# Grice-Lab/HmmUFOtu

Measured on AMD Instinct MI355X. Metric: reads placed/sec (whole node), gg_97_otus GTR+dGamma 250bp; HBM GB/s %peak, higher is better.
Workload: dtype f64; 1 GPU; gg_97_otus-scale synthetic DB (198643 nodes x 7682 CS columns, K=1400), GTR+dGamma(4), SE 250 bp amplicon reads, batch 8192 reads/step/GPU, 6 batches in flight, seeds in the reference's std::sort order (k_seed_refsort); seed_order=reference, message_window_cols=7682, parallelism=read-sharded x1

## Files before the change

### hmmufotu_amd/csrc/hu_common.h

```cpp
#pragma once
#include <hip/hip_runtime.h>
#include <stdint.h>
#include <string>
#include <functional>
#include <istream>
#include <ostream>
#include <vector>
#include <exception>
#include <mutex>
#include <thread>
#include "../../include/hmmufotu_amd.h"

#define HU_MAX_DGK 16
#define HU_READ_TILE 16
#define HU_MAX_INS 24
#define HU_NODE_PAD 256
#define HU_MIN_LOGLIK_EXP (-510.0)
#define HU_BRANCH_EPS 1e-5
#define HU_MAX_ITER 100

struct HuModelDev {
	int32_t type, dgK;
	double pi[4];
	double logpi[4];
	double U[16], U1[16], lam[4];
	double rate[HU_MAX_DGK];
};

struct HuDbDev {
	int32_t nNodes, nNodesPad, csLen, W, WQ, root;
	int64_t winStart, winLen;
	const uint4* planes;
	const int32_t* posCol;
	const unsigned long long* colPlanes;
	int32_t QM, pad0;
	const uint2* nodeCover;
	const int32_t* parent;
	const double* blen;
	const double* height;
	const double* up;
	const double* down;
	const int32_t* upK;
	const int32_t* downK;
	int32_t K, L;
	const double* EM;
	const double* EI;
	const double* T;
	const double* entryC;
	const double* exitC;
	const int32_t* p2cs;
	const double* Tt;
	const double* EMt;
	const double* EIt;
	const double* placeConst;
	int32_t rLo, rHi;
	const uint32_t* wideList;
};
__device__ inline bool hu_skip_width(const HuDbDev& db, int cols) { return db.rHi != 0 && (cols <= db.rLo || cols > db.rHi); }

struct HuRegion {
	int32_t j0, j1, i0, i1;
	int32_t withB;
	int32_t band;
	int32_t from, start, nIns, nDel;
	int64_t off;
	int64_t doff;
	int32_t ci0, cj0;
	int64_t coff;
};
// ... 75 lines not shown
```

### hmmufotu_amd/csrc/hu_engine.hip

```cpp
#include <algorithm>
#include <cmath>
#include <cstdio>
#include <cstring>
#include <limits>
#include <map>
#include <atomic>
#include <thread>
#include <memory>
#include <mutex>
#include <chrono>
#include <fstream>
#include <sstream>
#include <new>
#include <stdexcept>
#include <fcntl.h>
#include <unistd.h>
#include "hu_common.h"
#include "hu_kern_sep.h"
#include "hu_kern_align.h"
#include "hu_kern_tree.h"
#include "hu_kern_blk.h"
#include "hu_kern_refsort.h"
#include "hu_kern_rank.h"
#include "hu_kern_anneal.h"
// ... 90 lines not shown
			for(size_t i = 0; i < v.size(); ++i) if(v[i] == (void*) p) { v.erase(v.begin() + i); free(p); return; }
		}
		(void) hipHostFree(p);
	}
	static std::vector<void*>& pageable() { static std::vector<void*> v; return v; }
	static std::mutex& mtx() { static std::mutex m; return m; }
	template<class U> bool operator==(const PinnedAlloc<U>&) const { return true; }
	template<class U> bool operator!=(const PinnedAlloc<U>&) const { return false; }
};
template<class T> using PinnedVec = std::vector<T, PinnedAlloc<T>>;

template<class X> struct DBuf {
	X* p = nullptr; size_t cap = 0;
	int ensure(size_t n) {
		if(n <= cap) return HU_OK;
		if(p) (void) hipFree(p);
		p = nullptr; cap = 0;
		size_t want = n + n / 8 + 16;
		hipError_t e = hipMalloc((void**) &p, want * sizeof(X));
		if(e != hipSuccess) { hu_set_error("hipMalloc(%zu bytes) failed: %s", want * sizeof(X), hipGetErrorString(e)); return HU_ERR_NOMEM; }
		cap = want;
		return HU_OK;
	}
	void free_() { if(p) (void) hipFree(p); p = nullptr; cap = 0; }
	DBuf() = default;
	DBuf(const DBuf&) = delete;
	DBuf& operator=(const DBuf&) = delete;
	~DBuf() { free_(); }
};

struct hu_db {
	int device = 0;
	HuDbDev dev;
	double partialFrac = 0;
	HuModelDev mdl;
	hu_model_desc mdesc;
	HuProfileHost prof;
	std::vector<int32_t> parent, annoId;
	std::vector<double> blen, height, annoDist;
	std::vector<int8_t> seq;
	std::vector<std::string> annos, names;
	std::vector<void*> allocs;
	int64_t hbmBytes = 0;
	int32_t* dAnnoId = nullptr;
	double* dLlTab = nullptr;
	bool hasInvalidCode = false;
	std::mutex annealMu;
	bool annealReady = false;
	uint4* dInvPlane = nullptr;
	unsigned long long* dLeafMask = nullptr;
	std::vector<int32_t> colPos;
};

template<class X> static int dev_alloc(hu_db* db, X** p, size_t n) {
	size_t bytes = std::max<size_t>(n, 1) * sizeof(X);
	hipError_t e = hipMalloc((void**) p, bytes);
	if(e != hipSuccess) { hu_set_error("hipMalloc(%zu bytes) failed: %s", bytes, hipGetErrorString(e)); return HU_ERR_NOMEM; }
	db->allocs.push_back(*p);
	db->hbmBytes += (int64_t) bytes;
	return HU_OK;
}
template<class X> static int dev_upload(hu_db* db, X** p, const X* src, size_t n) {
	int rc = dev_alloc(db, p, n);
	if(rc != HU_OK) return rc;
	if(n) HIPCHK(hipMemcpy(*p, src, n * sizeof(X), hipMemcpyHostToDevice));
	return HU_OK;
// ... 108 lines not shown
				uint32_t* p0 = &pl[((size_t) q * 3 + 0) * np + i].x + w;
				uint32_t* p1 = &pl[((size_t) q * 3 + 1) * np + i].x + w;
				uint32_t* pv = &pl[((size_t) q * 3 + 2) * np + i].x + w;
				if(code & 1) *p0 |= bit;
				if(code & 2) *p1 |= bit;
				*pv |= bit;
			}
		}
		uint4* dp = nullptr;
		if((rc = dev_upload(db, &dp, pl.data(), cnt)) != HU_OK) return fail(rc);
		d.planes = dp;
		d.QM = (prof->K + 127) / 128;
		if(d.WQ > d.QM) {
			unsigned long long* cp = nullptr;
			if((rc = dev_alloc(db, &cp, (size_t)(d.WQ - d.QM) * 128 * 3 * (np / 64))) != HU_OK) return fail(rc);
			k_col_planes<<<dim3((unsigned)(np / 64), (unsigned)(d.WQ - d.QM)), 64>>>(d, cp);
			hipError_t e1 = hipGetLastError(), e2 = hipDeviceSynchronize();
			if(e1 != hipSuccess || e2 != hipSuccess) { hu_set_error("transposing the non-profile planes failed: %s", hipGetErrorString(e1 != hipSuccess ? e1 : e2)); return fail(HU_ERR_DEVICE); }
			d.colPlanes = cp;
		}
		{
			uint2* cv = nullptr;
			if((rc = dev_alloc(db, &cv, np)) != HU_OK) return fail(rc);
			k_node_cover<<<(unsigned)(np / 256), 256>>>(d, cv);
			hipError_t e1 = hipGetLastError(), e2 = hipDeviceSynchronize();
			if(e1 != hipSuccess || e2 != hipSuccess) { hu_set_error("node coverage intervals failed: %s", hipGetErrorString(e1 != hipSuccess ? e1 : e2)); return fail(HU_ERR_DEVICE); }
			d.nodeCover = cv;
			std::vector<uint2> hc((size_t) d.nNodes);
			if(hipMemcpy(hc.data(), cv, hc.size() * sizeof(uint2), hipMemcpyDeviceToHost) != hipSuccess) { hu_set_error("node coverage intervals: copy failed"); return fail(HU_ERR_DEVICE); }
			const uint32_t span = (uint32_t) std::min<int64_t>((int64_t) d.QM * 128, (int64_t) prof->K);
			size_t partial = 0;
			for(const uint2& c : hc) { const uint32_t f = c.x & 0xffffu, l = c.x >> 16; if(f > l || (l - f + 1) * 10u < span * 9u) ++partial; }
			db->partialFrac = d.nNodes ? (double) partial / d.nNodes : 0.0;
		}
	}
	{
		int32_t* p; double* q;
		if((rc = dev_upload(db, &p, db->parent.data(), (size_t) n)) != HU_OK) return fail(rc); d.parent = p;
		if((rc = dev_upload(db, &q, db->blen.data(), (size_t) n)) != HU_OK) return fail(rc); d.blen = q;
		if((rc = dev_upload(db, &q, db->height.data(), (size_t) n)) != HU_OK) return fail(rc); d.height = q;
	}
	{
		double *qu, *qd;
		const size_t cnt = (size_t) n * winLen * 4;
		if(tree->msgs_on_device) { qu = const_cast<double*>(tree->up); qd = const_cast<double*>(tree->down); db->hbmBytes += 2 * (int64_t) cnt * 8; }
		else {
			if((rc = dev_upload(db, &qu, tree->up, cnt)) != HU_OK) return fail(rc);
			if((rc = dev_upload(db, &qd, tree->down, cnt)) != HU_OK) return fail(rc);
		}
		int32_t *ku, *kd;
		const size_t ns = (size_t) n * winLen;
		if((rc = dev_alloc(db, &ku, ns)) != HU_OK) return fail(rc);
		if((rc = dev_alloc(db, &kd, ns)) != HU_OK) return fail(rc);
		(void) hipGetLastError();
		k_pack_msgs<<<(unsigned)((ns + 255) / 256), 256>>>(db->mdl, qu, ku, ns);
		k_pack_msgs<<<(unsigned)((ns + 255) / 256), 256>>>(db->mdl, qd, kd, ns);
		hipError_t e1 = hipGetLastError(), e2 = hipDeviceSynchronize();
		if(e1 != hipSuccess || e2 != hipSuccess) { hu_set_error("message packing failed: %s", hipGetErrorString(e1 != hipSuccess ? e1 : e2)); return fail(HU_ERR_DEVICE); }
		d.up = qu; d.down = qd; d.upK = ku; d.downK = kd;
	}
	{
		const int K = d.K;
		std::vector<double> T8((size_t)(K + 1) * 8, kInf);
		for(int k = 0; k <= K; ++k) for(int t = 0; t < 7; ++t) T8[(size_t) k * 8 + t] = db->prof.T7[(size_t) k * 7 + t];
		std::vector<int32_t> p2(K + 2, 0);
		for(int k = 0; k <= K; ++k) p2[k] = db->prof.p2cs[k];
// ... 562 lines not shown
		if(fill) {
			if(EM) memcpy(EM, vEM.data(), vEM.size() * 8); if(EI) memcpy(EI, vEI.data(), vEI.size() * 8);
			if(T) memcpy(T, vT.data(), vT.size() * 8); if(p2cs) memcpy(p2cs, vp.data(), vp.size() * 4);
			if(entryC) memcpy(entryC, prof.entryC.data(), prof.entryC.size() * 8);
			if(exitC) memcpy(exitC, prof.exitC.data(), prof.exitC.size() * 8);
		}
	}
	if(ptu_path) {
		HuTreeHost t;
		int rc = hu_read_ptu(ptu_path, t);
		if(rc != HU_OK) return rc;
		if(n_nodes) *n_nodes = t.n; if(root) *root = t.root; if(L && !hmm_path) *L = t.csLen;
		if(model) *model = t.model;
		if(fill) {
			if(parent) memcpy(parent, t.parent.data(), t.parent.size() * 4); if(blen) memcpy(blen, t.blen.data(), t.blen.size() * 8);
			if(seq) memcpy(seq, t.seq.data(), t.seq.size()); if(height) memcpy(height, t.height.data(), t.height.size() * 8);
			if(up) memcpy(up, t.up.data(), t.up.size() * 8); if(down) memcpy(down, t.down.data(), t.down.size() * 8);
		}
	}
	return HU_OK;
} catch(...) { return hu_catch_all("hu_files_parse"); }

extern "C" void hu_db_destroy(hu_db* db) try {
	if(!db) return;
	for(void* p : db->allocs) (void) hipFree(p);
	delete db;
} catch(...) { (void) hu_catch_all("hu_db_destroy"); }
extern "C" int hu_db_info(const hu_db* db, int32_t* K, int32_t* cs_len, int32_t* n_nodes, int32_t* root, int64_t* hbm_bytes) try {
	if(!db) return HU_ERR_ARG;
	if(K) *K = db->dev.K; if(cs_len) *cs_len = db->dev.csLen; if(n_nodes) *n_nodes = db->dev.nNodes;
	if(root) *root = db->dev.root; if(hbm_bytes) *hbm_bytes = db->hbmBytes;
	return HU_OK;
} catch(...) { return hu_catch_all("hu_db_info"); }
extern "C" int hu_db_get_profile(const hu_db* db, double* EM, double* EI, double* T, int32_t* p2cs, double* entry_cost, double* exit_cost) try {
	if(!db) return HU_ERR_ARG;
	const HuProfileHost& p = db->prof;
	if(EM) memcpy(EM, p.EM.data(), p.EM.size() * 8); if(EI) memcpy(EI, p.EI.data(), p.EI.size() * 8);
	if(T) memcpy(T, p.T7.data(), p.T7.size() * 8); if(p2cs) memcpy(p2cs, p.p2cs.data(), p.p2cs.size() * 4);
	if(entry_cost) memcpy(entry_cost, p.entryC.data(), p.entryC.size() * 8);
	if(exit_cost) memcpy(exit_cost, p.exitC.data(), p.exitC.size() * 8);
	return HU_OK;
} catch(...) { return hu_catch_all("hu_db_get_profile"); }
extern "C" int hu_db_get_tree(const hu_db* db, int32_t* parent, double* blen, int8_t* seq, double* height) try {
	if(!db) return HU_ERR_ARG;
	if(parent) memcpy(parent, db->parent.data(), db->parent.size() * 4); if(blen) memcpy(blen, db->blen.data(), db->blen.size() * 8);
	if(seq) memcpy(seq, db->seq.data(), db->seq.size()); if(height) memcpy(height, db->height.data(), db->height.size() * 8);
	return HU_OK;
} catch(...) { return hu_catch_all("hu_db_get_tree"); }
extern "C" const char* hu_db_get_annotation(const hu_db* db, int32_t node) try {
	if(!db || node < 0 || node >= (int32_t) db->annos.size()) return "";
	return db->annos[node].c_str();
} catch(...) { (void) hu_catch_all("hu_db_get_annotation"); return ""; }
extern "C" int hu_db_get_anno_dist(const hu_db* db, int32_t node, double* out) try {
	if(!db || !out || node < 0 || node >= (int32_t) db->annoDist.size()) return HU_ERR_ARG;
	*out = db->annoDist[node];
	return HU_OK;
} catch(...) { return hu_catch_all("hu_db_get_anno_dist"); }
extern "C" int hu_db_get_model(const hu_db* db, hu_model_desc* out) try { if(!db || !out) return HU_ERR_ARG; *out = db->mdesc; return HU_OK; } catch(...) { return hu_catch_all("hu_db_get_model"); }

__global__ void k_model_pr(HuModelDev mdl, int n, const double* __restrict__ t, double* __restrict__ P) {
	const int i = blockIdx.x * blockDim.x + threadIdx.x;
	if(i >= n) return;
	double E[4];
	for(int k = 0; k < 4; ++k) E[k] = exp(mdl.lam[k] * t[i]);
	for(int col = 0; col < 4; ++col) {
		double a[4], c[4];
// ... 566 lines not shown
	HuModelDev mdl;
	int rc = hu_model_prepare(model, &mdl);
	if(rc != HU_OK) return rc;
	HIPCHK(hipSetDevice(device));
	const int64_t L = cs_len;
	DBuf<double> dOut;
	if((rc = dOut.ensure((size_t) L)) != HU_OK) return rc;
	(void) hipGetLastError();
	k_tree_loglik<<<(unsigned)((L + 255) / 256), 256>>>(up_dev + (size_t) root * L * 4, L, mdl.pi[0], mdl.pi[1], mdl.pi[2], mdl.pi[3], dOut.p);
	HIPCHK(hipGetLastError());
	std::vector<double> own;
	if(!per_col) { own.resize((size_t) L); per_col = own.data(); }
	HIPCHK(hipMemcpy(per_col, dOut.p, (size_t) L * 8, hipMemcpyDeviceToHost));
	double s = 0;
	for(int64_t j = 0; j < L; ++j) s += per_col[j];
	*sum = s;
	return HU_OK;
} catch(...) { return hu_catch_all("hu_tree_loglik"); }


typedef HuPlaceRec HostPlace;

struct HuKnobs {
	int viterbi_hbm = 0;
	int viterbi_values = 0;
	int viterbi_mode = 0;
	int viterbi_dec1 = 0;
	int vw_diag = 0;
	int viterbi_force_redo = 0;
	int tile_unsorted = 0;
	int pairs32 = 0;
	int topk_fast_min = 16384;
	int topk_general = 0;
	int scan_pairs = 0;
	int streaming_sep = 0;
	int est_unsorted = 0, place_unsorted = 0;
	int xcd_map = 1;
	int est_var = 0, place_var = 0;
	int place_nosplit = 0;
	int place_lds_pad = 0;
	int est_lds_pad = 0;
	int vit_lds_pad = 0;
	int scan_lds_pad = 0;
	int trace = 0;
	int width_split = 1;
	int sort_seq = 0;
	int refsort_wgs = HU_RS_WGS_PER_CU * 256;
	int ref_nofuse = 0;
	int refsort_host = 0;
	int inject_fault = 0;
};
struct HuKnobEntry { const char* name; int HuKnobs::* field; };
static const HuKnobEntry kKnobs[] = {
	{"viterbi_hbm", &HuKnobs::viterbi_hbm}, {"viterbi_values", &HuKnobs::viterbi_values}, {"viterbi_mode", &HuKnobs::viterbi_mode},
	{"viterbi_dec1", &HuKnobs::viterbi_dec1}, {"vw_diag", &HuKnobs::vw_diag}, {"viterbi_force_redo", &HuKnobs::viterbi_force_redo},
	{"pairs32", &HuKnobs::pairs32}, {"tile_unsorted", &HuKnobs::tile_unsorted}, {"topk_fast_min", &HuKnobs::topk_fast_min}, {"scan_pairs", &HuKnobs::scan_pairs}, {"topk_general", &HuKnobs::topk_general}, {"streaming_sep", &HuKnobs::streaming_sep},
	{"est_unsorted", &HuKnobs::est_unsorted}, {"place_unsorted", &HuKnobs::place_unsorted}, {"xcd_map", &HuKnobs::xcd_map},
	{"est_var", &HuKnobs::est_var}, {"place_var", &HuKnobs::place_var}, {"place_nosplit", &HuKnobs::place_nosplit}, {"width_split", &HuKnobs::width_split},
	{"place_lds_pad", &HuKnobs::place_lds_pad}, {"est_lds_pad", &HuKnobs::est_lds_pad}, {"vit_lds_pad", &HuKnobs::vit_lds_pad}, {"scan_lds_pad", &HuKnobs::scan_lds_pad}, {"trace", &HuKnobs::trace}, {"inject_fault", &HuKnobs::inject_fault}, {"refsort_host", &HuKnobs::refsort_host}, {"ref_nofuse", &HuKnobs::ref_nofuse}, {"refsort_wgs", &HuKnobs::refsort_wgs}, {"sort_seq", &HuKnobs::sort_seq},
};
static void knobs_from_env(HuKnobs& k) {
	for(const HuKnobEntry& e : kKnobs) {
		std::string env = "HU_";
		for(const char* c = e.name; *c; ++c) env += (char) toupper(*c);
		const char* v = getenv(env.c_str());
		if(!v) continue;
		char* end = nullptr;
		const long x = strtol(v, &end, 10);
		k.*(e.field) = (end == v) ? 1 : (int) x;
	}
}

enum { ST_NONE = 0, ST_READS = 1, ST_ALIGNED = 2, ST_SEEDED = 3, ST_ESTIMATED = 4, ST_FILTERED = 5, ST_PLACED = 6, ST_FINISHED = 7 };

struct hu_batch {
	hu_db* db = nullptr;
	int maxReads = 0, n = 0, nSeq = 0, state = ST_NONE;
	bool paired = false, fromCodes = false, profile = false;
	HuKnobs knob;
	int maxBases = 1 << 30;
	bool fixedRoot = false;
	bool placesGiven = false;
	bool pair16 = false;
	int scanWidth = 0;
	int pairsKind = 0;
	int seedCap = HU_MAX_SEEDS;
	hipStream_t stream = nullptr;
	hipEvent_t ev[2 * HU_T_COUNT];
	bool evSet[HU_T_COUNT] = {false};
// ... 857 lines not shown
	const size_t n = (size_t) b->n;
	int rc;
	const int nBlk = d.nNodesPad / 256;
	const bool manyPartial = b->db->partialFrac > 0.02 && b->knob.scan_pairs != -1;
	if(o->seed_order != HU_SEED_ORDER_STABLE && o->seed_order != HU_SEED_ORDER_LIBSTDCXX) { hu_set_error("seed_order must be HU_SEED_ORDER_STABLE or HU_SEED_ORDER_LIBSTDCXX"); return HU_ERR_ARG; }
	const bool refOrder = o->seed_order == HU_SEED_ORDER_LIBSTDCXX;
	const bool dOnly = !refOrder && b->knob.scan_pairs != 1 && !manyPartial && o->max_height == INFINITY && nBlk >= 2 * o->max_nseed && nBlk <= 2048 && d.nNodes - 1 >= o->max_nseed;
	const bool narrow = !b->knob.pairs32 && b->maxBases <= 255;
	b->pair16 = !dOnly && narrow;
	b->pairsKind = dOnly ? 0 : (b->pair16 ? 16 : 32);
	b->scanWidth = dOnly ? (narrow ? 1 : 2) : 0;
	if((rc = b->dPairs.ensure(std::max<size_t>(n, 1) * d.nNodesPad / (dOnly ? (narrow ? 4 : 2) : (b->pair16 ? 2 : 1)))) != HU_OK) return rc;
	if((rc = b->dSeedCnt.ensure(n)) != HU_OK) return rc;
	if((rc = b->dSeedId.ensure(n * HU_MAX_SEEDS)) != HU_OK) return rc;
	if((rc = b->dSeedDN.ensure(n * HU_MAX_SEEDS)) != HU_OK) return rc;
	if((rc = b->dParDN.ensure(n * HU_MAX_SEEDS)) != HU_OK) return rc;
	uint32_t* bmin = nullptr;
	if(dOnly) {
		if((rc = b->dBmin.ensure(std::max<size_t>(n, 1) * nBlk + 16)) != HU_OK) return rc;
		if((rc = b->dRetry.ensure(n + 1)) != HU_OK) return rc;
		bmin = b->dBmin.p;
	}
	b->refFused = refOrder && n > 0 && ref_fused_l0(b, o, b->pair16);
	if(b->refFused) {
		if((rc = b->dRefPiv.ensure(n * 4)) != HU_OK || (rc = b->dRefL0.ensure(n * (size_t)(d.nNodesPad / 64) * 2)) != HU_OK) return rc;
		k_ref_pivots<<<(unsigned)((n + 63) / 64), 64, 0, b->stream>>>(d, read_planes(b), b->n, b->dRefPiv.p);
		HIPCHK(hipGetLastError());
	}
	uint32_t* stat = bmin && b->knob.trace ? bmin + n * nBlk : nullptr;
	if(stat) HIPCHK(hipMemsetAsync(stat, 0, 64, b->stream));
	(void) hipGetLastError();
	if(n) {
		const int tiles = (b->n + HU_READ_TILE - 1) / HU_READ_TILE;
		const dim3 grid(tiles, d.nNodesPad / 256);
		{
			Timer t(b, HU_T_SEED_PDIST);
			const dim3 grid4(tiles, (d.nNodesPad + 1023) / 1024);
			if(dOnly && narrow) k_seed_dscan4<uint8_t><<<grid4, 256, (size_t)(b->knob.scan_lds_pad > 0 && b->knob.scan_lds_pad <= 44 ? b->knob.scan_lds_pad : 0) * 1024, b->stream>>>(d, b->dRp.p, b->dTileQ.p, (uint8_t*) b->dPairs.p, b->dSlotRead.p, bmin, (const uint2*) b->dTileSpan.p);
			else if(dOnly) k_seed_dscan4<uint16_t><<<grid4, 256, 0, b->stream>>>(d, b->dRp.p, b->dTileQ.p, (uint16_t*) b->dPairs.p, b->dSlotRead.p, bmin, (const uint2*) b->dTileSpan.p);
			else if(b->refFused && b->pair16) k_seed_pdist2<uint16_t, true><<<grid, 256, 0, b->stream>>>(d, b->dRp.p, b->dTileQ.p, b->dTileIns.p, (uint16_t*) b->dPairs.p, b->dSlotRead.p, b->dRefPiv.p, b->dRefL0.p);
			else if(b->refFused) k_seed_pdist2<uint32_t, true><<<grid, 256, 0, b->stream>>>(d, b->dRp.p, b->dTileQ.p, b->dTileIns.p, b->dPairs.p, b->dSlotRead.p, b->dRefPiv.p, b->dRefL0.p);
			else if(b->pair16) k_seed_pdist2<uint16_t><<<grid, 256, 0, b->stream>>>(d, b->dRp.p, b->dTileQ.p, b->dTileIns.p, (uint16_t*) b->dPairs.p, b->dSlotRead.p);
			else k_seed_pdist2<uint32_t><<<grid, 256, 0, b->stream>>>(d, b->dRp.p, b->dTileQ.p, b->dTileIns.p, b->dPairs.p, b->dSlotRead.p);
		}
		{
			Timer t(b, HU_T_SEED_TOPK);
			if(dOnly) {
				int32_t* retry = b->dRetry.p;
				HIPCHK(hipMemsetAsync(retry, 0, 4, b->stream));
				#define TOPK_ARGS(T) d, (const T*) b->dPairs.p, bmin, read_planes(b), o->max_nseed, b->dSeedCnt.p, b->dSeedId.p, b->dSeedDN.p, b->dParDN.p, stat, retry
				if(narrow) { k_seed_topk_straight<uint8_t><<<b->n, 256, 0, b->stream>>>(TOPK_ARGS(uint8_t), b->knob.topk_general); k_seed_topk_d<uint8_t, true><<<std::min(b->n, 1024), 256, 0, b->stream>>>(TOPK_ARGS(uint8_t)); }
				else { k_seed_topk_straight<uint16_t><<<b->n, 256, 0, b->stream>>>(TOPK_ARGS(uint16_t), b->knob.topk_general); k_seed_topk_d<uint16_t, true><<<std::min(b->n, 1024), 256, 0, b->stream>>>(TOPK_ARGS(uint16_t)); }
				#undef TOPK_ARGS
			}
			else if(refOrder) { if((rc = seed_order_libstdcxx_device(b, o)) != HU_OK) return rc; }
			else {
				if(b->pair16) k_seed_topk<uint16_t><<<b->n, 256, 0, b->stream>>>(d, (const uint16_t*) b->dPairs.p, o->max_height, o->max_nseed, b->dSeedCnt.p, b->dSeedId.p, b->dSeedDN.p, b->knob.topk_fast_min);
				else k_seed_topk<uint32_t><<<b->n, 256, 0, b->stream>>>(d, b->dPairs.p, o->max_height, o->max_nseed, b->dSeedCnt.p, b->dSeedId.p, b->dSeedDN.p, b->knob.topk_fast_min);
				k_parent_pairs<<<((unsigned) n * HU_MAX_SEEDS + 255) / 256, 256, 0, b->stream>>>(d, b->n, b->dPairs.p, b->pair16 ? 1 : 0, b->dSeedCnt.p, b->dSeedId.p, b->dParDN.p);
			}
		}
		k_seed_drop_empty<<<(b->n + 255) / 256, 256, 0, b->stream>>>(b->n, b->dStart.p, b->dEnd.p, b->dSeedCnt.p);
		HIPCHK(hipGetLastError());
		if(stat) {
			uint32_t h[16];
			HIPCHK(hipMemcpyAsync(h, stat, 64, hipMemcpyDeviceToHost, b->stream)); HIPCHK(hu_wait(b->stream));
			fprintf(stderr, "[hu] top-k after the distance-only scan: %u of %zu reads on the block path (%.1f blocks, %.1f candidates per read), %u by the exact recomputation; "
				"%u of them through the general launch\n",
				h[0] + h[8], n, h[0] + h[8] ? (double) h[1] / (h[0] + h[8]) : 0.0, h[0] + h[8] ? (double) h[2] / (h[0] + h[8]) : 0.0, h[3], h[8]);
		}
	}
	b->seedCap = o->max_nseed;
	b->state = ST_SEEDED;
	return HU_OK;
} catch(...) { return hu_catch_all("hu_seed_batch"); }

// ... 1373 lines not shown
```

### hmmufotu_amd/csrc/hu_kern_sep.h

```cpp
#pragma once
#include "hu_common.h"

#define HU_TOPK_BINS 4097
#define HU_TOPK_CAP 4096

template<class PT> struct HuPair;
template<> struct HuPair<uint32_t> {
	static constexpr int PPV = 4;
	__device__ static inline uint32_t canon(uint32_t x) { return x; }
	__device__ static inline uint32_t pack(uint32_t c) { return c; }
	__device__ static inline void unpack(const uint4& v, uint32_t* o) { o[0] = v.x; o[1] = v.y; o[2] = v.z; o[3] = v.w; }
};
template<> struct HuPair<uint16_t> {
	static constexpr int PPV = 8;
	__device__ static inline uint32_t canon(uint32_t x) { return ((x >> 8) << 16) | (x & 0xffu); }
	__device__ static inline uint16_t pack(uint32_t c) { return (uint16_t)(((c >> 16) << 8) | (c & 0xffu)); }
	__device__ static inline void unpack(const uint4& v, uint32_t* o) {
		const uint32_t w[4] = {v.x, v.y, v.z, v.w};
#pragma unroll
		for(int e = 0; e < 8; ++e) o[e] = canon((w[e >> 1] >> ((e & 1) * 16)) & 0xffffu);
	}
};
__device__ inline uint32_t hu_pair_load(const void* pairs, size_t idx, int p16) {
	return p16 ? HuPair<uint16_t>::canon(((const uint16_t*) pairs)[idx]) : ((const uint32_t*) pairs)[idx];
}

__global__ __launch_bounds__(64) void k_col_planes(HuDbDev db, unsigned long long* __restrict__ col) {
	const int nb = blockIdx.x, q = db.QM + blockIdx.y, lane = threadIdx.x;
	const size_t np = (size_t) db.nNodesPad, npw = np / 64;
	const int node = nb * 64 + lane;
	for(int p = 0; p < 3; ++p) {
		const uint4 v = db.planes[((size_t) q * 3 + p) * np + node];
		const uint32_t w[4] = {v.x, v.y, v.z, v.w};
		for(int i = 0; i < 128; ++i) {
			const unsigned long long m = __ballot((w[i >> 5] >> (i & 31)) & 1u);
			if(lane == 0) col[(((size_t) blockIdx.y * 128 + i) * 3 + p) * npw + nb] = m;
		}
	}
}

__global__ __launch_bounds__(256) void k_node_cover(HuDbDev db, uint2* __restrict__ cover) {
	const int node = blockIdx.x * 256 + threadIdx.x;
	if(node >= db.nNodesPad) return;
	uint32_t f1 = 0xffffu, l1 = 0, f2 = 0xffffu, l2 = 0; bool any1 = false, any2 = false;
	for(int q = 0; q < db.WQ; ++q) {
		const uint4 v = db.planes[((size_t) q * 3 + 2) * db.nNodesPad + node];
		const uint32_t w[4] = {v.x, v.y, v.z, v.w};
		for(int k = 0; k < 4; ++k) {
			if(!w[k]) continue;
			const uint32_t lo = (uint32_t) q * 128 + k * 32 + (__ffs(w[k]) - 1), hi = (uint32_t) q * 128 + k * 32 + 31 - __clz(w[k]);
			if(q < db.QM) { if(!any1) { f1 = lo; any1 = true; } l1 = hi; }
			else { if(!any2) { f2 = lo; any2 = true; } l2 = hi; }
		}
	}
	cover[node] = make_uint2((any1 ? f1 : 0xffffu) | ((any1 ? l1 : 0u) << 16), (any2 ? f2 : 0xffffu) | ((any2 ? l2 : 0u) << 16));
}
__device__ inline bool hu_span_meets(uint32_t a, uint32_t b) {
	return (a & 0xffffu) <= (b >> 16) && (b & 0xffffu) <= (a >> 16) && (a & 0xffffu) <= (a >> 16) && (b & 0xffffu) <= (b >> 16);
}
__device__ inline bool hu_cover_meets(uint2 node, uint2 read) { return hu_span_meets(node.x, read.x) || hu_span_meets(node.y, read.y); }

template<int CTRL>
__device__ inline uint32_t dpp_min_full(uint32_t v) {
	const uint32_t o = (uint32_t) __builtin_amdgcn_mov_dpp((int) v, CTRL, 0xf, 0xf, true);
	return o < v ? o : v;
}
template<class PT, bool L0 = false>
__global__ __launch_bounds__(256) void k_seed_pdist2(HuDbDev db, const uint32_t* __restrict__ rp,
		const int32_t* __restrict__ tileQ, const int32_t* __restrict__ tileIns, PT* __restrict__ pairs, const int32_t* __restrict__ slotRead,
		uint32_t* __restrict__ piv = nullptr, unsigned long long* __restrict__ l0m = nullptr) {
	constexpr int T = HU_READ_TILE;
	__shared__ uint32_t acc[T][256];
	const int tile = blockIdx.x, tid = threadIdx.x;
	const int node = blockIdx.y * 256 + tid;
	const int32_t* __restrict__ ql = tileQ + (size_t) tile * (db.WQ + 1);
	const int32_t* __restrict__ til = tileIns + (size_t) tile * (T * HU_MAX_INS + 1);
	const int nq = ql[0], ne = til[0];
	uint32_t d[T], N[T];
#pragma unroll
	for(int t = 0; t < T; ++t) { d[t] = 0; N[t] = 0; }
	if(ne) {
#pragma unroll
		for(int t = 0; t < T; ++t) acc[t][tid] = 0;
	}
	const size_t np = (size_t) db.nNodesPad;
	for(int qi = 0; qi < nq; ++qi) {
		const int q = ql[1 + qi];
		const uint4 n0 = db.planes[((size_t) q * 3 + 0) * np + node], n1 = db.planes[((size_t) q * 3 + 1) * np + node], nv = db.planes[((size_t) q * 3 + 2) * np + node];
		const uint32_t* __restrict__ r = rp + (((size_t) tile * db.WQ + q) * T) * 16;
#pragma unroll
		for(int t = 0; t < T; ++t) {
			const uint32_t* rt = r + t * 16;
			uint32_t k, x;
			k = nv.x & rt[8];  x = ((n0.x ^ rt[0]) | (n1.x ^ rt[4])) & k; d[t] += __popc(x); N[t] += __popc(k);
			k = nv.y & rt[9];  x = ((n0.y ^ rt[1]) | (n1.y ^ rt[5])) & k; d[t] += __popc(x); N[t] += __popc(k);
			k = nv.z & rt[10]; x = ((n0.z ^ rt[2]) | (n1.z ^ rt[6])) & k; d[t] += __popc(x); N[t] += __popc(k);
			k = nv.w & rt[11]; x = ((n0.w ^ rt[3]) | (n1.w ^ rt[7])) & k; d[t] += __popc(x); N[t] += __popc(k);
		}
	}
	{
		const size_t npw = np / 64;
		const int nb = __builtin_amdgcn_readfirstlane(node >> 6), lane = tid & 63;
		for(int e = 0; e < ne; ++e) {
			const int ent = til[1 + e];
			const int t = ent >> 24, pos = (ent >> 2) & 0x3fffff, code = ent & 3;
			const unsigned long long* cp = db.colPlanes + ((size_t)(pos - db.QM * 128) * 3) * npw + nb;
			const unsigned long long W0 = cp[0], W1 = cp[npw], Wv = cp[2 * npw];
			const uint32_t valid = (uint32_t)(Wv >> lane) & 1u, nc = ((uint32_t)(W0 >> lane) & 1u) | (((uint32_t)(W1 >> lane) & 1u) << 1);
			const uint32_t add = valid | ((valid & (nc != (uint32_t) code ? 1u : 0u)) << 16);
			atomicAdd(&acc[t][tid], add);
		}
	}
	const bool counts = L0 && node < db.nNodes && node != db.root;
	bool zero = false;
#pragma unroll
	for(int t = 0; t < T; ++t) {
		const int read = slotRead[tile * T + t];
		if(read >= 0) {
			const uint32_t v = ((d[t] << 16) | N[t]) + (ne ? acc[t][tid] : 0u);
			pairs[(size_t) read * np + node] = HuPair<PT>::pack(v);
			if(L0) {
				const uint32_t pp = piv[(size_t) read * 4];
				const uint32_t a = (v >> 16) * (pp & 0xffffu), bb = (pp >> 16) * (v & 0xffffu);
				const unsigned long long mL = __ballot(counts && a >= bb), mR = __ballot(counts && bb >= a);
				if((tid & 63) == 0) *reinterpret_cast<ulonglong2*>(l0m + ((size_t) read * (np / 64) + (size_t)(node >> 6)) * 2) = make_ulonglong2(mL, mR);
				zero |= v == 0u;
			}
		}
	}
	if(L0 && __ballot(zero && counts)) {
#pragma unroll
		for(int t = 0; t < T; ++t) {
			const int read = slotRead[tile * T + t];
			if(read < 0) continue;
			const uint32_t v = ((d[t] << 16) | N[t]) + (ne ? acc[t][tid] : 0u);
			if(__ballot(counts && v == 0u) && (tid & 63) == 0) atomicOr(&piv[(size_t) read * 4 + 3], 1u);
		}
	}
}

template<class DT>
__global__ __launch_bounds__(256, 3) void k_seed_dscan4(HuDbDev db, const uint32_t* __restrict__ rp,
		const int32_t* __restrict__ tileQ, DT* __restrict__ dm, const int32_t* __restrict__ slotRead, uint32_t* __restrict__ bminD, const uint2* __restrict__ tileSpan) {
	constexpr int T = HU_READ_TILE, M = 4;
	constexpr uint32_t DMAX = (uint32_t)(DT) ~(DT) 0;
	static_assert(T == 16, "sixteen reads x sixteen dwords per quad = one dword per thread");
	__shared__ __attribute__((aligned(16))) uint32_t rpl2[2][T * 16];
	__shared__ __attribute__((aligned(16))) uint32_t mb[4][T][64];
	const int tile = blockIdx.x, tid = threadIdx.x, lane = tid & 63, wave = tid >> 6;
	const int node0 = blockIdx.y * (256 * M) + tid * M;
	const bool live = node0 < db.nNodesPad;
	const int nl = live ? node0 : 0;
	const int32_t* __restrict__ ql = tileQ + (size_t) tile * (db.WQ + 1);
	const int nq = ql[0];
	uint32_t d[T][M];
#pragma unroll
	for(int t = 0; t < T; ++t)
#pragma unroll
		for(int m = 0; m < M; ++m) d[t][m] = 0;
	const size_t np = (size_t) db.nNodesPad;
	for(int qi = 0; qi < nq; ++qi) {
		const int q = ql[1 + qi];
		const uint32_t mine = rp[((size_t) tile * db.WQ + q) * (T * 16) + tid];
		uint4 n0[M], n1[M], nv[M];
#pragma unroll
		for(int m = 0; m < M; ++m) {
			n0[m] = db.planes[((size_t) q * 3 + 0) * np + nl + m]; n1[m] = db.planes[((size_t) q * 3 + 1) * np + nl + m]; nv[m] = db.planes[((size_t) q * 3 + 2) * np + nl + m];
		}
// ... 1275 lines not shown
```

### hmmufotu_amd/engine.py

```python
from __future__ import annotations

import ctypes as C
import os
import subprocess

import numpy as np

_HERE = os.path.dirname(os.path.abspath(__file__))
LIB_PATH = os.environ.get("HU_LIB") or os.path.join(_HERE, "libhmmufotu_amd.so")
_LIB = None

HU_MAX_SEEDS = 64
T_NAMES = ["viterbi", "align_build", "seed_pdist", "seed_topk", "estimate", "place", "_6", "_7"]
MODE = {"global": 0, "local": 1, "ngcl": 2, "cgnl": 3}


class EngineError(RuntimeError):
    pass


class ProfileDesc(C.Structure):
    _fields_ = [("K", C.c_int32), ("L", C.c_int32), ("EM", C.POINTER(C.c_double)), ("EI", C.POINTER(C.c_double)),
                ("T", C.POINTER(C.c_double)), ("p2cs", C.POINTER(C.c_int32))]

# ... 1000 lines not shown
                    T=np.ascontiguousarray(hmm.T, np.float64), p2cs=np.ascontiguousarray(hmm.p2cs, np.int32),
                    parent=np.ascontiguousarray(parent, np.int32), blen=np.ascontiguousarray(blen, np.float64),
                    seq=np.ascontiguousarray(seq, np.int8), height=np.ascontiguousarray(height, np.float64))
        pd = ProfileDesc(int(hmm.K), int(hmm.L), _p(keep["EM"], C.c_double), _p(keep["EI"], C.c_double), _p(keep["T"], C.c_double),
                         _p(keep["p2cs"], C.c_int32))
        td = TreeDesc()
        td.n_nodes, td.cs_len = keep["seq"].shape
        td.parent = _p(keep["parent"], C.c_int32); td.blen = _p(keep["blen"], C.c_double); td.seq = _p(keep["seq"], C.c_int8)
        td.height = _p(keep["height"], C.c_double)
        if msgs_on_device:
            td.up = C.c_void_p(int(up)); td.down = C.c_void_p(int(down)); td.msgs_on_device = 1
        else:
            keep["up"] = np.ascontiguousarray(up, np.float64); keep["down"] = np.ascontiguousarray(down, np.float64)
            td.up = keep["up"].ctypes.data_as(C.c_void_p); td.down = keep["down"].ctypes.data_as(C.c_void_p)
        if anno_id is not None:
            keep["anno"] = np.ascontiguousarray(anno_id, np.int32); td.anno_id = _p(keep["anno"], C.c_int32)
        if anno_dist is not None:
            keep["annod"] = np.ascontiguousarray(anno_dist, np.float64); td.anno_dist = _p(keep["annod"], C.c_double)
        td.win_start = int(win_start); td.win_len = int(win_len)
        h = C.c_void_p()
        _chk(lib.hu_db_create(C.byref(pd), C.byref(td), C.byref(model), C.c_int(device), C.byref(h)))
        return cls(h, keep if msgs_on_device else None)

    @classmethod
    def from_synth(cls, db, device=0):
        md = model_desc(db.model.type_id, db.model.pi, db.model.par, db.dg_r if db.dg_k > 0 else None)
        return cls.from_arrays(db.hmm, db.parent, db.blen, db.seq, db.up, db.down, db.height, md, db.anno_id, db.anno_dist, device=device)

    @classmethod
    def load(cls, hmm_path: str, ptu_path: str, device=0, win_start=0, win_len=0):
        h = C.c_void_p()
        _chk(load_library().hu_db_load_window(hmm_path.encode(), ptu_path.encode(), C.c_int(device), C.c_int64(win_start), C.c_int64(win_len), C.byref(h)))
        return cls(h)

    def model_pr(self, t):
        t = np.ascontiguousarray(t, np.float64).ravel()
        P = np.zeros((len(t), 4, 4))
        _chk(load_library().hu_db_model_pr(self.h, C.c_int(len(t)), _p(t, C.c_double), _p(P, C.c_double)))
        return P

    def build_align_path(self, cs_start, cs_end, cs: str, cs_from, cs_to):
        out = np.zeros(6, np.int32)
        _chk(load_library().hu_build_align_path(self.h, C.c_int(cs_start), C.c_int(cs_end), cs.encode(), C.c_int(cs_from), C.c_int(cs_to),
                                                _p(out, C.c_int32)))
        return out

    def profile(self):
        K = self.K
        out = dict(EM=np.zeros((K + 1, 4)), EI=np.zeros((K + 1, 4)), T=np.zeros((K + 1, 7)), p2cs=np.zeros(K + 1, np.int32),
                   entry_cost=np.zeros(K + 1), exit_cost=np.zeros(K + 1))
        _chk(load_library().hu_db_get_profile(self.h, _p(out["EM"], C.c_double), _p(out["EI"], C.c_double), _p(out["T"], C.c_double),
                                              _p(out["p2cs"], C.c_int32), _p(out["entry_cost"], C.c_double), _p(out["exit_cost"], C.c_double)))
        return out

    def num_leaves(self) -> int:
        v = C.c_int64()
        _chk(load_library().hu_db_num_leaves(self.h, C.byref(v)))
        return int(v.value)

    def anneal(self, primers, identity=0.9, strand=3, batch=4096):
        max_dist = 1 - float(identity)
        if not max_dist >= 0:
            raise ValueError("-i|--identity must between 0 and 1")
        if strand not in (1, 2, 3):
            raise ValueError("-s|--strand must be 1, 2 or 3")
        opts = default_opts(align_mode="global")
# ... 498 lines not shown
```

### include/hmmufotu_amd.h

```cpp
#ifndef HMMUFOTU_AMD_H_
#define HMMUFOTU_AMD_H_

#include <stdint.h>

#ifdef __cplusplus
extern "C" {
#endif

typedef enum {
	HU_OK = 0,
	HU_ERR_ARG = -1,
	HU_ERR_DEVICE = -2,
	HU_ERR_IO = -3,
	HU_ERR_NOMEM = -4,
	HU_ERR_STATE = -5
} hu_status;

enum { HU_MODE_GLOBAL = 0, HU_MODE_LOCAL = 1, HU_MODE_NGCL = 2, HU_MODE_CGNL = 3 };
enum { HU_GTR = 0, HU_TN93 = 1, HU_HKY85 = 2, HU_F81 = 3, HU_K80 = 4, HU_JC69 = 5 };
enum { HU_PRIOR_UNIFORM = 0, HU_PRIOR_HEIGHT = 1 };

enum {
	HU_READ_OK = 1,
	HU_READ_INVALID = 0,
// ... 55 lines not shown
} hu_opts;
enum { HU_SEED_ORDER_STABLE = 0, HU_SEED_ORDER_LIBSTDCXX = 1 };

typedef struct {
	int32_t seq_start, seq_end, hmm_start, hmm_end, cs_start, cs_end;
	int32_t status;
	int32_t used_full;
	double cost;
} hu_align_rec;

typedef struct {
	int32_t c_node, p_node, a_node;
	int32_t n_cand;
	double wuv, ratio, wnr, loglik, height, q_place, q_taxon, anno_dist, est_loglik;
	double root_loglik;
} hu_place_rec;

void hu_default_opts(hu_opts* o);
const char* hu_last_error(void);
int hu_device_count(void);

int hu_db_create(const hu_profile_desc* prof, const hu_tree_desc* tree, const hu_model_desc* model,
		int device, hu_db** out);
int hu_db_load(const char* hmm_path, const char* ptu_path, int device, hu_db** out);
int hu_db_load_window(const char* hmm_path, const char* ptu_path, int device, int64_t win_start, int64_t win_len, hu_db** out);
int hu_profile_parse_text(const char* text, int64_t len, int32_t* K, int32_t* L, double* EM, double* EI, double* T, int32_t* p2cs);
int hu_model_parse_text(const char* text, int64_t len, hu_model_desc* out);
int hu_files_parse(const char* hmm_path, const char* ptu_path, int32_t* K, int32_t* L, int32_t* n_nodes, int32_t* root,
		double* EM, double* EI, double* T, int32_t* p2cs, double* entry_cost, double* exit_cost,
		int32_t* parent, double* blen, int8_t* seq, double* height, double* up, double* down, hu_model_desc* model, int fill);
int hu_model_spectral(const hu_model_desc* model, double* U, double* lam, double* U1);
void hu_db_destroy(hu_db* db);
int hu_db_info(const hu_db* db, int32_t* K, int32_t* cs_len, int32_t* n_nodes, int32_t* root, int64_t* hbm_bytes);
int hu_db_get_profile(const hu_db* db, double* EM, double* EI, double* T, int32_t* p2cs,
		double* entry_cost, double* exit_cost);
int hu_db_get_tree(const hu_db* db, int32_t* parent, double* blen, int8_t* seq, double* height);
int hu_db_get_model(const hu_db* db, hu_model_desc* out);
const char* hu_db_get_annotation(const hu_db* db, int32_t node);
int hu_db_model_pr(const hu_db* db, int n, const double* t, double* P );

int hu_tree_evaluate(int32_t n_nodes, int32_t cs_len, const int32_t* parent, const double* blen, int8_t* seq,
		const hu_model_desc* model, int device, int64_t win_start, int64_t win_len, double* up_dev, double* down_dev, double* height);

int hu_ptu_write(const char* path, const hu_tree_desc* tree, const char* const* names, const char* const* annos, const hu_model_desc* model,
		const char* model_text, double dg_alpha, const double* dg_breaks);

int hu_msa_encode_table(int8_t* out );
int hu_msa_stats(int device, int64_t n_seq, int64_t cs_len, const char* msa, int32_t* res_count, int32_t* gap_count,
		int32_t* start, int32_t* end, int32_t* len, double* seq_weight, double* res_wcount, double* gap_wcount);
int hu_tree_count_mutations(int device, int32_t n_nodes, int32_t cs_len, const int32_t* parent, const double* up_dev, int32_t* counts);
int hu_dg_model(int32_t K, double alpha, double* breaks, double* rates);
double hu_dg_estimate_shape(int64_t n, const double* X);

typedef struct hu_newick hu_newick;
int hu_newick_parse(const char* text, int64_t len, hu_newick** out);
void hu_newick_free(hu_newick* t);
int hu_newick_size(const hu_newick* t, int32_t* n_nodes);
int hu_newick_get(const hu_newick* t, int32_t* parent, double* blen, int32_t* child_off, int32_t* child_idx);
const char* hu_newick_name(const hu_newick* t, int32_t node);

typedef struct hu_tree_anno hu_tree_anno;
int hu_tree_annotate(int32_t n_nodes, const int32_t* parent, const double* blen, const char* const* names, const char* anno_text,
		int64_t anno_len, const char* root_name, hu_tree_anno** out);
void hu_tree_anno_free(hu_tree_anno* a);
const char* hu_tree_anno_name(const hu_tree_anno* a, int32_t node);
const char* hu_tree_anno_anno(const hu_tree_anno* a, int32_t node);
// ... 260 lines not shown
```

Before: 396,200 reads/s.

## Group fully covered nodes into whole waves so the pair scan skips validity planes

```diff
diff --git a/hmmufotu_amd/csrc/hu_common.h b/hmmufotu_amd/csrc/hu_common.h
--- a/hmmufotu_amd/csrc/hu_common.h
+++ b/hmmufotu_amd/csrc/hu_common.h
@@ -15,6 +15,9 @@
 #define HU_READ_TILE 16
 #define HU_MAX_INS 24
 #define HU_NODE_PAD 256
+#ifndef HU_SCAN_BLOCK
+#define HU_SCAN_BLOCK 256
+#endif
 #define HU_MIN_LOGLIK_EXP (-510.0)
 #define HU_BRANCH_EPS 1e-5
 #define HU_MAX_ITER 100
@@ -35,6 +38,8 @@
 	const unsigned long long* colPlanes;
 	int32_t QM, pad0;
 	const uint2* nodeCover;
+	const uint16_t* scanLane;
+	const uint8_t* scanWave;
 	const int32_t* parent;
 	const double* blen;
 	const double* height;
diff --git a/hmmufotu_amd/csrc/hu_engine.hip b/hmmufotu_amd/csrc/hu_engine.hip
--- a/hmmufotu_amd/csrc/hu_engine.hip
+++ b/hmmufotu_amd/csrc/hu_engine.hip
@@ -146,6 +146,8 @@
 struct hu_db {
 	int device = 0;
 	HuDbDev dev;
+	double scanCompleteShare = 0;
+	std::atomic<bool> scanShareSaid{false};
 	double partialFrac = 0;
 	HuModelDev mdl;
 	hu_model_desc mdesc;
@@ -320,6 +322,20 @@
 			size_t partial = 0;
 			for(const uint2& c : hc) { const uint32_t f = c.x & 0xffffu, l = c.x >> 16; if(f > l || (l - f + 1) * 10u < span * 9u) ++partial; }
 			db->partialFrac = d.nNodes ? (double) partial / d.nNodes : 0.0;
+		}
+		{
+			const size_t nblk = (np + HU_SCAN_BLOCK - 1) / HU_SCAN_BLOCK, nw = nblk * (HU_SCAN_BLOCK / 64);
+			uint16_t* ln = nullptr; uint8_t* wf = nullptr;
+			if((rc = dev_alloc(db, &ln, nblk * HU_SCAN_BLOCK)) != HU_OK || (rc = dev_alloc(db, &wf, nw)) != HU_OK) return fail(rc);
+			k_scan_groups<<<(unsigned) nblk, HU_SCAN_BLOCK>>>(d, ln, wf);
+			hipError_t e1 = hipGetLastError(), e2 = hipDeviceSynchronize();
+			if(e1 != hipSuccess || e2 != hipSuccess) { hu_set_error("the pair scan's lane map failed: %s", hipGetErrorString(e1 != hipSuccess ? e1 : e2)); return fail(HU_ERR_DEVICE); }
+			std::vector<uint8_t> hf(nw);
+			if(hipMemcpy(hf.data(), wf, nw, hipMemcpyDeviceToHost) != hipSuccess) { hu_set_error("the pair scan's lane map: copy failed"); return fail(HU_ERR_DEVICE); }
+			size_t full = 0;
+			for(uint8_t f : hf) full += f;
+			db->scanCompleteShare = (double) full / (double) nw;
+			d.scanLane = ln; d.scanWave = wf;
 		}
 	}
 	{
@@ -948,6 +964,15 @@
 	if(root) *root = db->dev.root; if(hbm_bytes) *hbm_bytes = db->hbmBytes;
 	return HU_OK;
 } catch(...) { return hu_catch_all("hu_db_info"); }
+extern "C" int hu_db_get_scan_groups(const hu_db* db, int32_t* block, int32_t* n_slots, uint16_t* lane_node, uint8_t* wave_complete) try {
+	if(!db) return HU_ERR_ARG;
+	const size_t nblk = ((size_t) db->dev.nNodesPad + HU_SCAN_BLOCK - 1) / HU_SCAN_BLOCK, ns = nblk * HU_SCAN_BLOCK;
+	if(block) *block = HU_SCAN_BLOCK; if(n_slots) *n_slots = (int32_t) ns;
+	HIPCHK(hipSetDevice(db->device));
+	if(lane_node) HIPCHK(hipMemcpy(lane_node, db->dev.scanLane, ns * sizeof(uint16_t), hipMemcpyDeviceToHost));
+	if(wave_complete) HIPCHK(hipMemcpy(wave_complete, db->dev.scanWave, ns / 64, hipMemcpyDeviceToHost));
+	return HU_OK;
+} catch(...) { return hu_catch_all("hu_db_get_scan_groups"); }
 extern "C" int hu_db_get_profile(const hu_db* db, double* EM, double* EI, double* T, int32_t* p2cs, double* entry_cost, double* exit_cost) try {
 	if(!db) return HU_ERR_ARG;
 	const HuProfileHost& p = db->prof;
@@ -1580,6 +1605,7 @@
 	int pairs32 = 0;
 	int topk_fast_min = 16384;
 	int topk_general = 0;
+	int scan_ungrouped = 0;
 	int scan_pairs = 0;
 	int streaming_sep = 0;
 	int est_unsorted = 0, place_unsorted = 0;
@@ -1602,7 +1628,7 @@
 static const HuKnobEntry kKnobs[] = {
 	{"viterbi_hbm", &HuKnobs::viterbi_hbm}, {"viterbi_values", &HuKnobs::viterbi_values}, {"viterbi_mode", &HuKnobs::viterbi_mode},
 	{"viterbi_dec1", &HuKnobs::viterbi_dec1}, {"vw_diag", &HuKnobs::vw_diag}, {"viterbi_force_redo", &HuKnobs::viterbi_force_redo},
-	{"pairs32", &HuKnobs::pairs32}, {"tile_unsorted", &HuKnobs::tile_unsorted}, {"topk_fast_min", &HuKnobs::topk_fast_min}, {"scan_pairs", &HuKnobs::scan_pairs}, {"topk_general", &HuKnobs::topk_general}, {"streaming_sep", &HuKnobs::streaming_sep},
+	{"pairs32", &HuKnobs::pairs32}, {"tile_unsorted", &HuKnobs::tile_unsorted}, {"topk_fast_min", &HuKnobs::topk_fast_min}, {"scan_pairs", &HuKnobs::scan_pairs}, {"scan_ungrouped", &HuKnobs::scan_ungrouped}, {"topk_general", &HuKnobs::topk_general}, {"streaming_sep", &HuKnobs::streaming_sep},
 	{"est_unsorted", &HuKnobs::est_unsorted}, {"place_unsorted", &HuKnobs::place_unsorted}, {"xcd_map", &HuKnobs::xcd_map},
 	{"est_var", &HuKnobs::est_var}, {"place_var", &HuKnobs::place_var}, {"place_nosplit", &HuKnobs::place_nosplit}, {"width_split", &HuKnobs::width_split},
 	{"place_lds_pad", &HuKnobs::place_lds_pad}, {"est_lds_pad", &HuKnobs::est_lds_pad}, {"vit_lds_pad", &HuKnobs::vit_lds_pad}, {"scan_lds_pad", &HuKnobs::scan_lds_pad}, {"trace", &HuKnobs::trace}, {"inject_fault", &HuKnobs::inject_fault}, {"refsort_host", &HuKnobs::refsort_host}, {"ref_nofuse", &HuKnobs::ref_nofuse}, {"refsort_wgs", &HuKnobs::refsort_wgs}, {"sort_seq", &HuKnobs::sort_seq},
@@ -2526,16 +2552,21 @@
 	(void) hipGetLastError();
 	if(n) {
 		const int tiles = (b->n + HU_READ_TILE - 1) / HU_READ_TILE;
-		const dim3 grid(tiles, d.nNodesPad / 256);
+		const dim3 grid(tiles, (d.nNodesPad + HU_SCAN_BLOCK - 1) / HU_SCAN_BLOCK);
+		HuDbDev ds = d;
+		if(b->knob.scan_ungrouped == 1) { ds.scanLane = nullptr; ds.scanWave = nullptr; }
+		else if(b->knob.scan_ungrouped == 2) ds.scanWave = nullptr;
+		if(!dOnly && b->knob.trace && !b->knob.scan_ungrouped && !b->db->scanShareSaid.exchange(true))
+			fprintf(stderr, "[hu] pair scan: %.1f %% of the waves hold complete nodes only (blocks of %d node ids) and skip the compared-site count\n", 100.0 * b->db->scanCompleteShare, HU_SCAN_BLOCK);
 		{
 			Timer t(b, HU_T_SEED_PDIST);
 			const dim3 grid4(tiles, (d.nNodesPad + 1023) / 1024);
 			if(dOnly && narrow) k_seed_dscan4<uint8_t><<<grid4, 256, (size_t)(b->knob.scan_lds_pad > 0 && b->knob.scan_lds_pad <= 44 ? b->knob.scan_lds_pad : 0) * 1024, b->stream>>>(d, b->dRp.p, b->dTileQ.p, (uint8_t*) b->dPairs.p, b->dSlotRead.p, bmin, (const uint2*) b->dTileSpan.p);
 			else if(dOnly) k_seed_dscan4<uint16_t><<<grid4, 256, 0, b->stream>>>(d, b->dRp.p, b->dTileQ.p, (uint16_t*) b->dPairs.p, b->dSlotRead.p, bmin, (const uint2*) b->dTileSpan.p);
-			else if(b->refFused && b->pair16) k_seed_pdist2<uint16_t, true><<<grid, 256, 0, b->stream>>>(d, b->dRp.p, b->dTileQ.p, b->dTileIns.p, (uint16_t*) b->dPairs.p, b->dSlotRead.p, b->dRefPiv.p, b->dRefL0.p);
-			else if(b->refFused) k_seed_pdist2<uint32_t, true><<<grid, 256, 0, b->stream>>>(d, b->dRp.p, b->dTileQ.p, b->dTileIns.p, b->dPairs.p, b->dSlotRead.p, b->dRefPiv.p, b->dRefL0.p);
-			else if(b->pair16) k_seed_pdist2<uint16_t><<<grid, 256, 0, b->stream>>>(d, b->dRp.p, b->dTileQ.p, b->dTileIns.p, (uint16_t*) b->dPairs.p, b->dSlotRead.p);
-			else k_seed_pdist2<uint32_t><<<grid, 256, 0, b->stream>>>(d, b->dRp.p, b->dTileQ.p, b->dTileIns.p, b->dPairs.p, b->dSlotRead.p);
+			else if(b->refFused && b->pair16) k_seed_pdist2<uint16_t, true><<<grid, HU_SCAN_BLOCK, 0, b->stream>>>(ds, b->dRp.p, b->dTileQ.p, b->dTileIns.p, (uint16_t*) b->dPairs.p, b->dSlotRead.p, b->dRefPiv.p, b->dRefL0.p);
+			else if(b->refFused) k_seed_pdist2<uint32_t, true><<<grid, HU_SCAN_BLOCK, 0, b->stream>>>(ds, b->dRp.p, b->dTileQ.p, b->dTileIns.p, b->dPairs.p, b->dSlotRead.p, b->dRefPiv.p, b->dRefL0.p);
+			else if(b->pair16) k_seed_pdist2<uint16_t><<<grid, HU_SCAN_BLOCK, 0, b->stream>>>(ds, b->dRp.p, b->dTileQ.p, b->dTileIns.p, (uint16_t*) b->dPairs.p, b->dSlotRead.p);
+			else k_seed_pdist2<uint32_t><<<grid, HU_SCAN_BLOCK, 0, b->stream>>>(ds, b->dRp.p, b->dTileQ.p, b->dTileIns.p, b->dPairs.p, b->dSlotRead.p);
 		}
 		{
 			Timer t(b, HU_T_SEED_TOPK);
diff --git a/hmmufotu_amd/csrc/hu_kern_sep.h b/hmmufotu_amd/csrc/hu_kern_sep.h
--- a/hmmufotu_amd/csrc/hu_kern_sep.h
+++ b/hmmufotu_amd/csrc/hu_kern_sep.h
@@ -55,6 +55,29 @@
 	}
 	cover[node] = make_uint2((any1 ? f1 : 0xffffu) | ((any1 ? l1 : 0u) << 16), (any2 ? f2 : 0xffffu) | ((any2 ? l2 : 0u) << 16));
 }
+__global__ __launch_bounds__(HU_SCAN_BLOCK) void k_scan_groups(HuDbDev db, uint16_t* __restrict__ laneNode, uint8_t* __restrict__ waveFlag) {
+	constexpr int NB = HU_SCAN_BLOCK, NW = NB / 64;
+	__shared__ uint32_t cnt[NW];
+	const int tid = threadIdx.x, node = blockIdx.x * NB + tid, wave = tid >> 6;
+	bool complete = node < db.nNodes;
+	for(int q = 0; q < db.WQ && complete; ++q) {
+		const uint4 v = db.planes[((size_t) q * 3 + 2) * db.nNodesPad + node];
+		const uint32_t w[4] = {v.x, v.y, v.z, v.w};
+		for(int k = 0; k < 4; ++k) {
+			const int left = db.csLen - (q * 128 + k * 32);
+			const uint32_t want = left >= 32 ? 0xffffffffu : left <= 0 ? 0u : (1u << left) - 1u;
+			complete = complete && (w[k] & want) == want;
+		}
+	}
+	const unsigned long long m = __ballot(complete);
+	if((tid & 63) == 0) cnt[wave] = (uint32_t) __popcll(m);
+	__syncthreads();
+	uint32_t before = (uint32_t) __popcll(m & ((1ull << (tid & 63)) - 1ull)), total = 0;
+	for(int w = 0; w < NW; ++w) { if(w < wave) before += cnt[w]; total += cnt[w]; }
+	const uint32_t slot = complete ? before : total + ((uint32_t) tid - before);
+	laneNode[(size_t) blockIdx.x * NB + slot] = (uint16_t) tid;
+	if(tid < NW) waveFlag[(size_t) blockIdx.x * NW + tid] = (uint32_t)(tid + 1) * 64u <= total ? 1 : 0;
+}
 __device__ inline bool hu_span_meets(uint32_t a, uint32_t b) {
 	return (a & 0xffffu) <= (b >> 16) && (b & 0xffffu) <= (a >> 16) && (a & 0xffffu) <= (a >> 16) && (b & 0xffffu) <= (b >> 16);
 }
@@ -66,27 +89,52 @@
 	return o < v ? o : v;
 }
 template<class PT, bool L0 = false>
-__global__ __launch_bounds__(256) void k_seed_pdist2(HuDbDev db, const uint32_t* __restrict__ rp,
+__global__ __launch_bounds__(HU_SCAN_BLOCK) void k_seed_pdist2(HuDbDev db, const uint32_t* __restrict__ rp,
 		const int32_t* __restrict__ tileQ, const int32_t* __restrict__ tileIns, PT* __restrict__ pairs, const int32_t* __restrict__ slotRead,
 		uint32_t* __restrict__ piv = nullptr, unsigned long long* __restrict__ l0m = nullptr) {
-	constexpr int T = HU_READ_TILE;
-	__shared__ uint32_t acc[T][256];
+	constexpr int T = HU_READ_TILE, NB = HU_SCAN_BLOCK, NW = NB / 64;
+	static_assert(NB % HU_NODE_PAD == 0 && (NW & (NW - 1)) == 0, "whole padding units per block, a power of two of waves");
+	__shared__ uint32_t acc[T][NB];
 	const int tile = blockIdx.x, tid = threadIdx.x;
-	const int node = blockIdx.y * 256 + tid;
+	const size_t np = (size_t) db.nNodesPad;
+	const int own = blockIdx.y * NB + tid;
+	const bool live = NB == HU_NODE_PAD || (size_t) own < np;
+	const bool grouped = db.scanLane != nullptr;
+	const uint32_t rot = ((blockIdx.y * gridDim.x + blockIdx.x) * 0x9E3779B1u) >> 28;
+	const int slot = (tid + 64 * (int)(rot & (NW - 1))) & (NB - 1);
+	const int ln = grouped ? (int) db.scanLane[(size_t) blockIdx.y * NB + slot] : tid;
+	const bool gapless = db.scanWave != nullptr && db.scanWave[(size_t) blockIdx.y * NW + __builtin_amdgcn_readfirstlane(slot >> 6)] != 0;
+	const int snode = NB == HU_NODE_PAD || (size_t)(blockIdx.y * NB + ln) < np ? blockIdx.y * NB + ln : 0;
 	const int32_t* __restrict__ ql = tileQ + (size_t) tile * (db.WQ + 1);
 	const int32_t* __restrict__ til = tileIns + (size_t) tile * (T * HU_MAX_INS + 1);
 	const int nq = ql[0], ne = til[0];
 	uint32_t d[T], N[T];
 #pragma unroll
-	for(int t = 0; t < T; ++t) { d[t] = 0; N[t] = 0; }
-	if(ne) {
-#pragma unroll
-		for(int t = 0; t < T; ++t) acc[t][tid] = 0;
-	}
-	const size_t np = (size_t) db.nNodesPad;
-	for(int qi = 0; qi < nq; ++qi) {
+	for(int t = 0; t < T; ++t) { d[t] = 0; N[t] = 0; acc[t][tid] = 0; }
+	if(gapless) {
+		uint32_t Ns[T];
+#pragma unroll
+		for(int t = 0; t < T; ++t) Ns[t] = 0;
+		for(int qi = 0; qi < nq; ++qi) {
+			const int q = ql[1 + qi];
+			const uint4 n0 = db.planes[((size_t) q * 3 + 0) * np + snode], n1 = db.planes[((size_t) q * 3 + 1) * np + snode];
+			const uint32_t* __restrict__ r = rp + (((size_t) tile * db.WQ + q) * T) * 16;
+#pragma unroll
+			for(int t = 0; t < T; ++t) {
+				const uint32_t* rt = r + t * 16;
+				d[t] += __popc(((n0.x ^ rt[0]) | (n1.x ^ rt[4])) & rt[8]);
+				d[t] += __popc(((n0.y ^ rt[1]) | (n1.y ^ rt[5])) & rt[9]);
+				d[t] += __popc(((n0.z ^ rt[2]) | (n1.z ^ rt[6])) & rt[10]);
+				d[t] += __popc(((n0.w ^ rt[3]) | (n1.w ^ rt[7])) & rt[11]);
+				Ns[t] += __popc(rt[8]) + __popc(rt[9]) + __popc(rt[10]) + __popc(rt[11]);
+			}
+		}
+#pragma unroll
+		for(int t = 0; t < T; ++t) N[t] = Ns[t];
+	}
+	else for(int qi = 0; qi < nq; ++qi) {
 		const int q = ql[1 + qi];
-		const uint4 n0 = db.planes[((size_t) q * 3 + 0) * np + node], n1 = db.planes[((size_t) q * 3 + 1) * np + node], nv = db.planes[((size_t) q * 3 + 2) * np + node];
+		const uint4 n0 = db.planes[((size_t) q * 3 + 0) * np + snode], n1 = db.planes[((size_t) q * 3 + 1) * np + snode], nv = db.planes[((size_t) q * 3 + 2) * np + snode];
 		const uint32_t* __restrict__ r = rp + (((size_t) tile * db.WQ + q) * T) * 16;
 #pragma unroll
 		for(int t = 0; t < T; ++t) {
@@ -98,9 +146,9 @@
 			k = nv.w & rt[11]; x = ((n0.w ^ rt[3]) | (n1.w ^ rt[7])) & k; d[t] += __popc(x); N[t] += __popc(k);
 		}
 	}
-	{
+	if(live) {
 		const size_t npw = np / 64;
-		const int nb = __builtin_amdgcn_readfirstlane(node >> 6), lane = tid & 63;
+		const int nb = __builtin_amdgcn_readfirstlane(own >> 6), lane = tid & 63;
 		for(int e = 0; e < ne; ++e) {
 			const int ent = til[1 + e];
 			const int t = ent >> 24, pos = (ent >> 2) & 0x3fffff, code = ent & 3;
@@ -111,13 +159,19 @@
 			atomicAdd(&acc[t][tid], add);
 		}
 	}
+	__syncthreads();
+#pragma unroll
+	for(int t = 0; t < T; ++t) atomicAdd(&acc[t][ln], (d[t] << 16) | N[t]);
+	__syncthreads();
+	if(!live) return;
+	const int node = own;
 	const bool counts = L0 && node < db.nNodes && node != db.root;
 	bool zero = false;
 #pragma unroll
 	for(int t = 0; t < T; ++t) {
 		const int read = slotRead[tile * T + t];
 		if(read >= 0) {
-			const uint32_t v = ((d[t] << 16) | N[t]) + (ne ? acc[t][tid] : 0u);
+			const uint32_t v = acc[t][tid];
 			pairs[(size_t) read * np + node] = HuPair<PT>::pack(v);
 			if(L0) {
 				const uint32_t pp = piv[(size_t) read * 4];
@@ -133,7 +187,7 @@
 		for(int t = 0; t < T; ++t) {
 			const int read = slotRead[tile * T + t];
 			if(read < 0) continue;
-			const uint32_t v = ((d[t] << 16) | N[t]) + (ne ? acc[t][tid] : 0u);
+			const uint32_t v = acc[t][tid];
 			if(__ballot(counts && v == 0u) && (tid & 63) == 0) atomicOr(&piv[(size_t) read * 4 + 3], 1u);
 		}
 	}
diff --git a/hmmufotu_amd/engine.py b/hmmufotu_amd/engine.py
--- a/hmmufotu_amd/engine.py
+++ b/hmmufotu_amd/engine.py
@@ -1056,6 +1056,14 @@
         h = C.c_void_p()
         _chk(load_library().hu_db_load_window(hmm_path.encode(), ptu_path.encode(), C.c_int(device), C.c_int64(win_start), C.c_int64(win_len), C.byref(h)))
         return cls(h)
+
+    def scan_groups(self):
+        lib = load_library()
+        blk = C.c_int32(); ns = C.c_int32()
+        _chk(lib.hu_db_get_scan_groups(self.h, C.byref(blk), C.byref(ns), None, None))
+        lane = np.zeros(ns.value, np.uint16); wave = np.zeros(ns.value // 64, np.uint8)
+        _chk(lib.hu_db_get_scan_groups(self.h, None, None, _p(lane, C.c_uint16), _p(wave, C.c_uint8)))
+        return blk.value, lane, wave
 
     def model_pr(self, t):
         t = np.ascontiguousarray(t, np.float64).ravel()
diff --git a/include/hmmufotu_amd.h b/include/hmmufotu_amd.h
--- a/include/hmmufotu_amd.h
+++ b/include/hmmufotu_amd.h
@@ -111,6 +111,7 @@
 int hu_model_spectral(const hu_model_desc* model, double* U, double* lam, double* U1);
 void hu_db_destroy(hu_db* db);
 int hu_db_info(const hu_db* db, int32_t* K, int32_t* cs_len, int32_t* n_nodes, int32_t* root, int64_t* hbm_bytes);
+int hu_db_get_scan_groups(const hu_db* db, int32_t* block, int32_t* n_slots, uint16_t* lane_node, uint8_t* wave_complete);
 int hu_db_get_profile(const hu_db* db, double* EM, double* EI, double* T, int32_t* p2cs,
 		double* entry_cost, double* exit_cost);
 int hu_db_get_tree(const hu_db* db, int32_t* parent, double* blen, int8_t* seq, double* height);
```

New measurement: 397,400 reads/s, median of 6. About the same (+0.3%).
